# kingdomseed/Deep-Fake-Audio-Classifier

Measured on AMD Instinct MI355X. Metric: utterances/sec fwd (2D-CNN, [B,T=321,F=180]) at 1/2/4/8 GPU; dev EER parity, higher is better.
Workload: dtype bf16; 1 GPU; BASELINE configs[1]: CNN2D eval forward, synthetic [256,321,180] per GPU, bf16 storage / fp32 accumulate, strided view of stored [B,180,321]; batch_per_gpu=256, T=321, F=180, parallelism=utterance-sharded x1, no collective

## Files before the change

deep-fake-audio-classifier_amd/csrc/api.hip:

```cpp
#include <stdlib.h>

#include <algorithm>

#include "dfa_checks.h"

using namespace dfa;

template <typename Fill>
static int stage_ragged_table(dfa_ctx* ctx, const int32_t* lengths, int B, size_t words, void* dst, Fill fill_rest) {
  if (words > ctx->ragged_cap) {
    for (auto& e : ctx->ragged_done)
      if (e) DFA_HIP_CHECK(ctx, hipEventSynchronize(e));
    if (ctx->ragged_host) DFA_HIP_CHECK(ctx, hipHostFree(ctx->ragged_host));
    ctx->ragged_host = nullptr;
    ctx->ragged_cap = 0;
    const size_t cap = std::max(words, (size_t)4 * 256);
    DFA_HIP_CHECK(ctx, hipHostMalloc((void**)&ctx->ragged_host, dfa_ctx::kRaggedSlots * cap * sizeof(int32_t), hipHostMallocDefault));
    ctx->ragged_cap = cap;
  }
  const int slot = ctx->ragged_slot;
  ctx->ragged_slot = (slot + 1) % dfa_ctx::kRaggedSlots;
  if (!ctx->ragged_done[slot]) DFA_HIP_CHECK(ctx, hipEventCreateWithFlags(&ctx->ragged_done[slot], hipEventDisableTiming));
  else DFA_HIP_CHECK(ctx, hipEventSynchronize(ctx->ragged_done[slot]));
  int32_t* tab = ctx->ragged_host + slot * ctx->ragged_cap;
// ... 97 lines not shown

namespace {
__global__ __launch_bounds__(256) void poison_lds_kernel(unsigned pattern, unsigned* sink) {
  extern __shared__ unsigned lds_words[];
  constexpr int N = 160 * 1024 / 4;
  for (int i = threadIdx.x; i < N; i += 256) lds_words[i] = pattern;
  __syncthreads();
  __builtin_amdgcn_s_sleep(127);
  if (lds_words[(threadIdx.x * 97 + blockIdx.x) % N] != pattern) sink[0] = 1;
}
hipError_t launch_poison_lds(dfa_ctx* ctx, unsigned half) {
  hipError_t e = hipSetDevice(ctx->device);
  if (e == hipSuccess) e = hipFuncSetAttribute((const void*)poison_lds_kernel, hipFuncAttributeMaxDynamicSharedMemorySize, 160 * 1024);
  if (e != hipSuccess) return e;
  half &= 0xffffu;
  hipLaunchKernelGGL(poison_lds_kernel, dim3(2048), dim3(256), 160 * 1024, ctx->stream, half | (half << 16), (unsigned*)ctx->zero_page);
  return hipGetLastError();
}
}

namespace {
enum OptionKind { OPT_FLAG, OPT_INT };
struct Option { const char* name; int dfa_ctx::*field; OptionKind kind; };
const Option kOptions[] = {
    {"time_split", &dfa_ctx::time_split, OPT_INT},
    {"conv1_bwd_fused", &dfa_ctx::conv1_bwd_fused, OPT_FLAG}, {"dgrad_m16", &dfa_ctx::dgrad_m16, OPT_FLAG},
    {"conv1_mfma", &dfa_ctx::conv1_mfma, OPT_FLAG}, {"cae_enc1_mfma", &dfa_ctx::cae_enc1_mfma, OPT_FLAG},
    {"cae_enc_dma", &dfa_ctx::cae_enc_dma, OPT_FLAG}, {"cae_dgrad_mfma", &dfa_ctx::cae_dgrad_mfma, OPT_FLAG},
    {"cae_conv_stats", &dfa_ctx::cae_conv_stats, OPT_FLAG}, {"cae_bwd_fold", &dfa_ctx::cae_bwd_fold, OPT_FLAG},
    {"cae_enc4_wide", &dfa_ctx::cae_enc4_wide, OPT_FLAG}, {"cae_dec_fused", &dfa_ctx::cae_dec_fused, OPT_FLAG},
    {"block3_m16", &dfa_ctx::block3_m16, OPT_FLAG}, {"fuse_conv1", &dfa_ctx::fuse_conv1, OPT_FLAG},
    {"fuse_blocks123", &dfa_ctx::fuse_blocks123, OPT_FLAG}, {"persist123", &dfa_ctx::persist123, OPT_FLAG},
    {"lds_pipe", &dfa_ctx::lds_pipe, OPT_FLAG}, {"carry_a1", &dfa_ctx::carry_a1, OPT_FLAG},
    {"phase123", &dfa_ctx::phase123, OPT_FLAG},
};
}

int dfa_ctx_set_option(dfa_ctx* ctx, const char* name, int value) {
  if (!ctx || !name) return DFA_E_NULL_PTR;
  if (strcmp(name, "poison_lds") == 0) {
    hipError_t e = launch_poison_lds(ctx, (unsigned)value);
    return e == hipSuccess ? DFA_OK : fail(ctx, DFA_E_HIP, "poison_lds: %s", hipGetErrorString(e));
  }
  if (strcmp(name, "train_conv_variant") == 0) { set_train_conv_variant(value); return DFA_OK; }
  if (strcmp(name, "wgrad_variant") == 0) { set_wgrad_variant(value); return DFA_OK; }
  if (strcmp(name, "clock_probe") == 0) {
    if (value && !ctx->clock_buf) {
      DFA_HIP_CHECK(ctx, hipSetDevice(ctx->device));
      DFA_HIP_CHECK(ctx, hipMalloc((void**)&ctx->clock_buf, 1024 * 2 * sizeof(long long)));
    }
    if (value) DFA_HIP_CHECK(ctx, hipMemsetAsync(ctx->clock_buf, 0, 1024 * 2 * sizeof(long long), ctx->stream));
    ctx->clock_probe = value ? 1 : 0;
    return DFA_OK;
  }
  if (strcmp(name, "cnn1d_train_x3") == 0) { ctx->cnn1d_train_x3 = (value < 0 || value > 3) ? 1 : value; return DFA_OK; }
  if (strcmp(name, "cnn1d_fused") == 0) { ctx->cnn1d_fused = value < 0 ? 0 : (value > 2 ? 1 : value); return DFA_OK; }
  if (strcmp(name, "conv_dma") == 0) { ctx->conv_dma = value < 0 ? -1 : value; return DFA_OK; }
  for (const Option& o : kOptions)
    if (strcmp(name, o.name) == 0) { ctx->*o.field = (o.kind == OPT_FLAG) ? (value ? 1 : 0) : value; return DFA_OK; }
  return fail(ctx, DFA_E_UNSUPPORTED, "unknown option '%s'", name);
}

int dfa_ctx_timing_enable(dfa_ctx* ctx, int enable) {
  if (!ctx) return DFA_E_NULL_PTR;
  ctx->timing = (enable == 1) ? 0xffffffffu : (unsigned)enable;
  return DFA_OK;
}
// ... 82 lines not shown
```

deep-fake-audio-classifier_amd/csrc/cnn1d_api.hip:

```cpp
#include "dfa_checks.h"
#include "trace.h"

using namespace dfa;

namespace {

struct Cnn1dPlan {
  size_t h1_off, h2_off, pooled_off, total;
};

Cnn1dPlan plan_cnn1d(int B, int T) {
  Cnn1dPlan p;
  size_t off = 0;
  p.h1_off = off;
  off = align_up(off + (size_t)B * 32 * T * sizeof(float), 256);
  p.h2_off = off;
  off = align_up(off + (size_t)B * 64 * T * sizeof(float), 256);
  p.pooled_off = off;
  off = align_up(off + (size_t)B * 128 * sizeof(float), 256);
  p.total = off;
  return p;
}

int cnn1d_forward_front(dfa_ctx* ctx, bool ragged, bool have_ptrs, int x_dtype, int B, int T, int F) {
// ... 57 lines not shown
}

int dfa_cnn1d_forward(dfa_ctx* ctx, const void* x, int x_dtype, int B, int T, int F, int64_t stride_b, int64_t stride_t,
                      int64_t stride_f, float* logits, void* workspace, size_t workspace_bytes) {
  TraceRange trace_("dfa_cnn1d_forward");
  if (!ctx) return DFA_E_NULL_PTR;
  Cnn1dState& m = ctx->cnn1d;
  DFA_TRY(cnn1d_forward_front(ctx, false, x && logits && workspace, x_dtype, B, T, F));
  const Cnn1dPlan pl = plan_cnn1d(B, T);
  DFA_TRY(check_workspace(ctx, workspace, workspace_bytes, pl.total, false));
  char* ws = (char*)workspace;
  float *h1 = (float*)(ws + pl.h1_off), *h2 = (float*)(ws + pl.h2_off), *pooled = (float*)(ws + pl.pooled_off);
  hipStream_t s = ctx->stream;
  const bool off32 = stride_t >= 0 && stride_f >= 0 && (int64_t)(F - 1) * stride_f + (int64_t)(T - 1) * stride_t < ((int64_t)1 << 31);
  if (ctx->cnn1d_fused == 1 && cnn1d_fused_x3_supports(x, stride_b, stride_t, stride_f, T, F)) {
    ScopedSlot ts(ctx, 4);
    DFA_HIP_CHECK(ctx, launch_cnn1d_fused_x3((const float*)x, m.wx[0], m.b[0], m.wx[1], m.b[1], m.wx[2], m.b[2], m.p[18], m.p[19], logits, B, T, F,
                                             s, ctx->clock_probe ? ctx->clock_buf : nullptr));
    return DFA_OK;
  }
  if (ctx->cnn1d_fused && cnn1d_fused_supports(T) && off32) {
    ScopedSlot ts(ctx, 4);
    DFA_HIP_CHECK(ctx, launch_cnn1d_fused((const float*)x, stride_b, stride_t, stride_f, m.wp[0], m.b[0], m.wp[1], m.b[1], m.wp[2], m.b[2],
                                          m.p[18], m.p[19], logits, B, T, F, s, ctx->clock_probe ? ctx->clock_buf : nullptr));
    return DFA_OK;
  }
  { ScopedSlot ts(ctx, 4);
    DFA_HIP_CHECK(ctx, launch_conv1d((const float*)x, stride_b, stride_f, stride_t, m.w[0], m.b[0], h1, B, F, 32, T, false, s)); }
  { ScopedSlot ts(ctx, 5);
    DFA_HIP_CHECK(ctx, launch_conv1d(h1, (int64_t)32 * T, T, 1, m.w[1], m.b[1], h2, B, 32, 64, T, false, s)); }
  { ScopedSlot ts(ctx, 6);
    DFA_HIP_CHECK(ctx, launch_conv1d(h2, (int64_t)64 * T, T, 1, m.w[2], m.b[2], pooled, B, 64, 128, T, true, s)); }
  { ScopedSlot ts(ctx, 7);
    DFA_HIP_CHECK(ctx, launch_linear(pooled, m.p[18], m.p[19], logits, B, 128, s)); }
  return DFA_OK;
}

int dfa_cnn1d_forward_ragged(dfa_ctx* ctx, const void* x, int x_dtype, int B, int T_max, int F, int64_t stride_b, int64_t stride_t,
                             int64_t stride_f, const int32_t* lengths, float* logits, void* workspace, size_t workspace_bytes) {
  TraceRange trace_("dfa_cnn1d_forward_ragged");
  if (!ctx) return DFA_E_NULL_PTR;
  Cnn1dState& m = ctx->cnn1d;
  DFA_TRY(cnn1d_forward_front(ctx, true, x && logits && workspace && lengths, x_dtype, B, T_max, F));
  if (T_max < 3) return fail(ctx, DFA_E_BAD_SHAPE, "T_max=%d is too short: the ragged cnn1d kernel needs T >= 3", T_max);
  DFA_TRY(check_lengths(ctx, lengths, B, 3, T_max));
  if (stride_t != 1)
    return fail(ctx, DFA_E_UNSUPPORTED, "the ragged cnn1d forward takes the channel-major storage only: stride_t=%lld, needs 1", (long long)stride_t);
  if ((F & 3) != 0) return fail(ctx, DFA_E_UNSUPPORTED, "the ragged cnn1d forward needs F %% 4 == 0 (got F=%d)", F);
  DFA_TRY(check_channel_major(ctx, "ragged cnn1d forward", "stride_f", x, stride_b, stride_f, T_max));
  if ((int64_t)F * stride_f >= ((int64_t)1 << 31))
    return fail(ctx, DFA_E_UNSUPPORTED, "the ragged cnn1d forward needs F * stride_f < 2^31 (got %d * %lld)", F, (long long)stride_f);
  if (ctx->cnn1d_fused != 1)
    return fail(ctx, DFA_E_UNSUPPORTED, "the ragged cnn1d forward needs the default option cnn1d_fused=1 (got %d)", ctx->cnn1d_fused);
  if (cnn1d_ragged_segments(3, F, nullptr, nullptr, nullptr, nullptr, 0) < 1)
    return fail(ctx, DFA_E_UNSUPPORTED, "F=%d: the layer-1 weights leave no LDS for a time window", F);
  DFA_TRY(refuse_capture(ctx, "forward"));
  DFA_TRY(check_workspace(ctx, workspace, workspace_bytes, cnn1d_workspace_bytes(B, T_max, true)));
  DFA_TRY(stage_ragged_lengths(ctx, lengths, B, workspace));
  ScopedSlot ts(ctx, 4);
  DFA_HIP_CHECK(ctx, launch_cnn1d_ragged_x3((const float*)x, stride_b, stride_f, (const int*)workspace, m.wx[0], m.b[0], m.wx[1], m.b[1], m.wx[2],
                                            m.b[2], m.p[18], m.p[19], logits, B, T_max, F, ctx->stream,
                                            ctx->clock_probe ? ctx->clock_buf : nullptr));
  return DFA_OK;
}

int dfa_cnn1d_ragged_segments(int T, int F, int* starts, int* lens, int* owned_lo, int* owned_hi, int cap) {
  return cnn1d_ragged_segments(T, F, starts, lens, owned_lo, owned_hi, cap);
// ... 8 lines not shown
```

deep-fake-audio-classifier_amd/csrc/cnn1d_train_api.hip:

```cpp
#include "train_host.h"
#include "trace.h"

using namespace dfa;

namespace {

struct Train1dPlan {
  size_t z[3], h[2], pooled, dpooled, dz[3], dh[2], stats, sums, partial, total;
};

Train1dPlan plan_train1d(int B, int T, int F) {
  Train1dPlan p;
  Bump take;
  const int C[3] = {32, 64, 128};
  for (int l = 0; l < 3; ++l) p.z[l] = take((size_t)B * C[l] * T * 4);
  for (int l = 0; l < 2; ++l) p.h[l] = take((size_t)B * C[l] * T * 4);
  p.pooled = take((size_t)B * 128 * 4);
  p.dpooled = take((size_t)B * 128 * 4);
  for (int l = 0; l < 3; ++l) p.dz[l] = take((size_t)B * C[l] * T * 4);
  for (int l = 0; l < 2; ++l) p.dh[l] = take((size_t)B * C[l] * T * 4);
  p.stats = take((32 + 64 + 128) * 3 * 4);
  p.sums = take((32 + 64 + 128) * 2 * 4);
  const size_t nch = (size_t)cm_chunks(B);
  size_t pb = nch * 128 * 2 * 4;
// ... 84 lines not shown
  m.train_drop = dc; m.train_B = B; m.train_T = T;
  m.train_ragged = lengths ? 1 : 0; m.train_frames = frames;
  char* ws = (char*)workspace;
  float* partial = (float*)(ws + pl.partial);
  const int C[3] = {32, 64, 128}, Cin[3] = {F, 32, 64};
  const int nch = cm_chunks(B);
  for (int l = 0; l < 3; ++l) {
    float* z = (float*)(ws + pl.z[l]);
    const float* const* q = p + 6 * l;
    if (l == 0) {
      if (x3 && conv1d_x3_supports((const float*)x, stride_b, stride_f, stride_t, z, T, F, 32, terms))
        DFA_HIP_CHECK(ctx, launch_conv1d_x3((const float*)x, stride_b, m.wx3[0], q[1], z, B, F, 32, T, terms, s, x3, aug, lens));
      else
        DFA_HIP_CHECK(ctx, launch_conv1d((const float*)x, stride_b, stride_f, stride_t, q[0], q[1], z, B, F, 32, T, false, s, false, aug, lens));
    } else {
      const float* hin = (const float*)(ws + pl.h[l - 1]);
      if (x3 && conv1d_x3_supports(hin, (int64_t)Cin[l] * T, T, 1, z, T, Cin[l], C[l], terms))
        DFA_HIP_CHECK(ctx, launch_conv1d_x3(hin, (int64_t)Cin[l] * T, m.wx3[l], q[1], z, B, Cin[l], C[l], T, terms, s, x3));
      else
        DFA_HIP_CHECK(ctx, launch_conv1d(hin, (int64_t)Cin[l] * T, T, 1, q[0], q[1], z, B, Cin[l], C[l], T, false, s, false));
    }
    BnStats st = st1d(ws, pl, l);
    const bool shifted = !ctx->bn_sync.fn;
    DFA_HIP_CHECK(ctx, launch_cm_stats(z, partial, B, C[l], T, s, lens, shifted));
    DFA_TRY(finalize_bn_stats(ctx, partial, nch, C[l], frames, st, update_running_stats ? (float*)q[4] : nullptr,
                              update_running_stats ? (float*)q[5] : nullptr, momentum, nullptr, shifted ? z : nullptr, T));
    if (l < 2) {
      dc.layer = 1 + l;
      DFA_HIP_CHECK(ctx, launch_cm_bn_relu_drop(z, st.mean, st.invstd, q[2], q[3], (float*)(ws + pl.h[l]), B, C[l], T, dc, s, lens));
    } else {
      DFA_HIP_CHECK(ctx, launch_cm_bn_relu_meant(z, st.mean, st.invstd, q[2], q[3], (float*)(ws + pl.pooled), B, 128, T, s, lens));
    }
  }
  DFA_HIP_CHECK(ctx, launch_linear((const float*)(ws + pl.pooled), p[18], p[19], logits, B, 128, s));
  return DFA_OK;
}

int cnn1d_backward_impl(dfa_ctx* ctx, int ragged, const void* x, int x_dtype, int B, int T, int F, int64_t stride_b, int64_t stride_t,
                        int64_t stride_f, const float* dlogits, float* const* grads, int ngrads, void* workspace,
                        size_t workspace_bytes) {
  Cnn1dState& m = ctx->cnn1d;
  Train1dPlan pl;
  DFA_TRY(check_backward(ctx, {ragged ? "dfa_cnn1d_backward_ragged" : "dfa_cnn1d_backward",
                               ragged ? "dfa_cnn1d_forward_train_ragged" : "dfa_cnn1d_forward_train", "cnn1d", 14, "dlogits", true},
                         m.train_packed && m.train_B == B && m.train_T == T && m.train_ragged == ragged, x, x_dtype, dlogits, grads, ngrads,
                         workspace, workspace_bytes, [&] { return (pl = plan_train1d(B, T, F)).total + (ragged ? ragged1d_tab_bytes(B) : 0); }));
  if (ragged && ctx->bn_sync.fn)
    return fail(ctx, DFA_E_UNSUPPORTED, "the ragged cnn1d training step cannot run under synchronised BatchNorm (dfa_ctx_set_bn_sync is armed)");
  char* ws = (char*)workspace;
  const int* lens = ragged ? (const int*)(ws + pl.total) : nullptr;
  float* partial = (float*)(ws + pl.partial);
  const float* const* p = m.p;
  hipStream_t s = ctx->stream;
  DropCfg dc = m.train_drop;
  const int C[3] = {32, 64, 128}, Cin[3] = {F, 32, 64};
  float* dpooled = (float*)(ws + pl.dpooled);
  DFA_HIP_CHECK(ctx, launch_linear_bwd(dlogits, p[18], (const float*)(ws + pl.pooled), dpooled, grads[12], grads[13], B, 128, s));
  for (int l = 2; l >= 0; --l) {
    const float* const* q = p + 6 * l;
    BnStats st = st1d(ws, pl, l);
    float* sm = sums1d(ws, pl, l);
    float* dz = (float*)(ws + pl.dz[l]);
    const float* up = (l == 2) ? dpooled : (const float*)(ws + pl.dh[l]);
    dc.layer = 1 + l;
    DFA_HIP_CHECK(ctx, launch_cm_bn_bwd(l == 2 ? 0 : 1, (const float*)(ws + pl.z[l]), st.mean, st.invstd, q[2], q[3], up, partial, sm, dz,
                                        B, C[l], T, dc, s, ctx->bn_sync.fn ? &ctx->bn_sync : nullptr, lens, m.train_frames));
    DFA_HIP_CHECK(ctx, launch_split_sums(sm, grads[4 * l + 2], grads[4 * l + 3], C[l], s));
// ... 75 lines not shown
```

deep-fake-audio-classifier_amd/csrc/cnn2d_api.hip:

```cpp
#include <algorithm>

#include "dfa_checks.h"
#include "trace.h"

using namespace dfa;

namespace {

constexpr int kMaxSeg = 4;

constexpr int kSlots = 512;
constexpr int kSlotsSplit2 = 768;
constexpr int kSlotsSplit3 = 256;
constexpr int kStripCols = c123::SW;
constexpr int kStripColsMfma = 32;

int seg_iters_for(int niter, int nwg, int slots, int period, int forced) {
  if (forced == 0 || niter <= period) return 0;
  int seg;
  if (forced > 0) seg = (niter + forced - 1) / forced;
  else {
    if (nwg >= slots) return 0;
    seg = (int)(((long long)niter * nwg + slots - 1) / slots);
  }
// ... 199 lines not shown
    a.in = a1; a.wpack = m.c2.wpack; a.bias = m.c2.bias; a.out = a2; a.emb = nullptr;
    a.B = B; a.H = pl.H1; a.W = F; a.COUT = 64; a.inv_h = 0.f; a.relu = 1; a.zero_page = ctx->zero_page;
    a.seg_iters = pl.seg12;
    if (prec == DFA_PREC_BF16X3) DFA_HIP_CHECK(ctx, launch_cnn2d_block2_split(a, s, ctx->lds_pipe));
    else DFA_HIP_CHECK(ctx, launch_cnn2d_block2(prec, a, s, ctx->conv_dma, ctx->lds_pipe));
  }
  if (pl.path != DFA_CNN2D_PATH_CONV123) {
    ScopedSlot ts(ctx, 2);
    ConvArgs a{};
    a.in = a2; a.wpack = m.c3.wpack; a.bias = m.c3.bias; a.out = nullptr; a.emb = emb;
    a.B = B; a.H = pl.H2; a.W = F; a.COUT = 128; a.inv_h = 1.0f / (float)pl.H2; a.relu = 1; a.zero_page = ctx->zero_page;
    a.chunk_iters = pl.chunk3;
    a.seg_iters = pl.seg3;
    if (pl.seg3) {
      a.emb_seg_stride = (size_t)B * 128 * F;
      a.emb = (float*)(ws + pl.emb_off) + a.emb_seg_stride;
    }
    if (prec == DFA_PREC_BF16X3) {
      DFA_HIP_CHECK(ctx, launch_cnn2d_block3_split(a, s, ctx->lds_pipe));
    } else if (prec == DFA_PREC_BF16 && ctx->block3_m16) {
      a.wpack = m.c3_m16;
      a.clock_stamps = ctx->clock_probe ? ctx->clock_buf : nullptr;
      DFA_HIP_CHECK(ctx, launch_cnn2d_block3_m16(a, s, ctx->lds_pipe));
    } else {
      DFA_HIP_CHECK(ctx, launch_cnn2d_block3(prec, a, s, ctx->conv_dma, ctx->lds_pipe));
    }
  }
  {
    ScopedSlot ts(ctx, 3);
    if (pl.nseg3 > 1) {
      const size_t n = (size_t)B * 128 * F;
      DFA_HIP_CHECK(ctx, launch_emb_reduce((const float*)(ws + pl.emb_off) + n, pl.nseg3, n, n, 1.0f / (float)pl.H2, emb, s));
    }
    DFA_HIP_CHECK(ctx, launch_linear(emb, m.p[18], m.p[19], logits, B, 128 * F, s));
  }
  return DFA_OK;
}

int dfa_cnn2d_forward_ragged(dfa_ctx* ctx, const void* x, int x_dtype, int B, int T_max, int F, int64_t stride_b, int64_t stride_t,
                             int64_t stride_f, const int32_t* lengths, float* logits, float* embedding, void* workspace,
                             size_t workspace_bytes) {
  TraceRange trace_("dfa_cnn2d_forward_ragged");
  if (!ctx) return DFA_E_NULL_PTR;
  Cnn2dState& m = ctx->cnn2d;
  DFA_TRY(cnn2d_forward_front(ctx, true, x && logits && workspace && lengths, x_dtype, B, T_max, F));
  DFA_TRY(check_lengths(ctx, lengths, B, 4, T_max));
  const int prec = m.prepared_prec;
  if (prec != DFA_PREC_BF16)
    return fail(ctx, DFA_E_UNSUPPORTED, "the ragged forward has kernels for precision bf16 only (prepared: %d)", prec);
  if (!ctx->fuse_conv1 || !ctx->block3_m16)
    return fail(ctx, DFA_E_UNSUPPORTED, "the ragged forward needs the default options fuse_conv1=1 and block3_m16=1");
  DFA_TRY(refuse_capture(ctx, "forward"));
  const Cnn2dForwardPlan pl = plan_for(ctx, B, T_max, F, prec, true);
  DFA_TRY(cnn2d_forward_buffers(ctx, workspace, workspace_bytes, pl.total, embedding));
  char* ws = (char*)workspace;
  const int* dtab = (const int*)(ws + pl.tab_off);
  hipStream_t s = ctx->stream;
  int nseg3 = 1;
  std::vector<int32_t> extra((size_t)2 * B);
  for (int b = 0; b < B; ++b) {
    const int h2 = lengths[b] / 4, niter3 = (h2 + 1) / 2, chunk = chunk3_for(niter3);
    const float inv_h = 1.0f / (float)h2;
    memcpy(&extra[b], &inv_h, 4);
    extra[B + b] = chunk;
    nseg3 = std::max(nseg3, (niter3 + chunk - 1) / chunk);
  }
  DFA_TRY(stage_ragged_lengths_extra(ctx, lengths, B, extra.data(), extra.size(), ws + pl.tab_off));
  const RaggedTab rt{dtab, B};
  void* a2 = ws + pl.a2_off;
  float* emb = embedding ? embedding : (float*)(ws + pl.emb_off);
  {
    ScopedSlot ts(ctx, 1);
    DFA_HIP_CHECK(ctx, launch_conv12_ragged(x, x_dtype, stride_b, stride_t, stride_f, m.c1pack, m.c1bias, m.c2.wpack, m.c2.bias, a2,
                                            B, T_max, F, dtab, s, ctx->lds_pipe, pl.seg12));
  }
  {
    ScopedSlot ts(ctx, 2);
    ConvArgs a{};
    a.in = a2; a.wpack = m.c3_m16; a.bias = m.c3.bias; a.out = nullptr; a.emb = emb;
    a.B = B; a.H = pl.H2; a.W = F; a.COUT = 128; a.relu = 1; a.zero_page = ctx->zero_page;
    a.chunk_iters = 1;
    if (pl.split3) {
      a.seg_iters = pl.seg3;
      a.emb_seg_stride = (size_t)B * 128 * F;
      a.emb = (float*)(ws + pl.emb_off) + a.emb_seg_stride;
    }
    DFA_HIP_CHECK(ctx, launch_cnn2d_block3_m16_ragged(a, rt, nseg3, s, ctx->lds_pipe));
  }
  {
    ScopedSlot ts(ctx, 3);
    if (pl.split3) {
      const size_t n = (size_t)B * 128 * F;
      DFA_HIP_CHECK(ctx, launch_emb_reduce_ragged((const float*)(ws + pl.emb_off) + n, n, 128 * F, dtab, B, emb, s));
    }
    DFA_HIP_CHECK(ctx, launch_linear(emb, m.p[18], m.p[19], logits, B, 128 * F, s));
  }
  return DFA_OK;
}

}
```

deep-fake-audio-classifier_amd/csrc/conv123_body.h:

```cpp
#ifndef DFA_CONV123_BODY_SCOPE
#error "conv123_body.h holds kernel bodies: include it only from conv123_fused.hip, conv123_persist.hip, conv123_carry.hip and conv123_phase.hip"
#endif
#ifndef DFA_CONV123_BODY_H
#define DFA_CONV123_BODY_H
#include "dfa_internal.h"
#ifdef DFA_STAMPS
#include <algorithm>
#include <climits>
#include <cstdio>
#include <vector>
#endif

#ifndef DFA_C123_PRIO
#define DFA_C123_PRIO 0
#endif
#ifndef DFA_C123_CBAR
#define DFA_C123_CBAR 4
#endif
#ifndef DFA_C123_CARRY
#define DFA_C123_CARRY 0
#endif

namespace dfa {

// ... 365 lines not shown
    c1_issue(st, j);
    if constexpr (PIPE) asm volatile("s_waitcnt lgkmcnt(0)" : "+v"(st.w0), "+v"(st.w1), "+v"(st.w2), "+v"(st.w3));
    c1_mfma(st, std::integral_constant<int, 0>{});
    c1_relu(st, j, std::integral_constant<int, 0>{});
    c1_store(st, ringblk, std::integral_constant<int, 0>{});
    c1_mfma(st, std::integral_constant<int, 1>{});
    c1_relu(st, j, std::integral_constant<int, 1>{});
    c1_store(st, ringblk, std::integral_constant<int, 1>{});
  };
  auto produce_fresh = [&](int j, int ringblk) {
#if DFA_C123_CARRY
    produce_cy(j, ringblk, std::true_type{});
    return;
#endif
    C1State st;
    c1_issue(st, j);
    if constexpr (PIPE) asm volatile("s_waitcnt lgkmcnt(0)" : "+v"(st.w0), "+v"(st.w1), "+v"(st.w2), "+v"(st.w3));
    c1_mfma(st, std::integral_constant<int, 0>{});
    c1_relu(st, j, std::integral_constant<int, 0>{});
    c1_store_fresh(st, ringblk, std::integral_constant<int, 0>{});
    c1_mfma(st, std::integral_constant<int, 1>{});
    c1_relu(st, j, std::integral_constant<int, 1>{});
    c1_store_fresh(st, ringblk, std::integral_constant<int, 1>{});
  };

  const int col = f0 - 1 + r;
  bool col_ok = col >= 0 && col < W;
  const int a2_dst = r * CPB;
  const int a2_sw = r & 6;
  auto lds_drain = [&]() { if constexpr (PIPE) asm volatile("s_waitcnt lgkmcnt(0)" ::: "memory"); };
  auto barrier = [&]() { lds_drain(); __syncthreads(); };

  barrier();
  x_load(0); x_store(0);
  x_load(1); x_store(1);
  barrier();
  produce_now(0, 0);
  produce_now(1, 1);
  barrier();
  x_load(2); x_store(0);
  barrier();

  auto unit = [&](auto ph_c, auto rp_c, int it) {
    constexpr int PH = decltype(ph_c)::value, RPI = decltype(rp_c)::value;
    f32x16_t acc0, acc1;
    constexpr int NR = 12 * NKG;
    constexpr int S_RELU0 = 9 * NKG + 2;
    constexpr int S_BAR = 4;
    constexpr int C_MFMA = 5, C_XLOAD = 7, C_RELU = 10, C_MFMA1 = 11, C_STORE = 13, C_RELU1 = 17, C_XSTORE = 19, C_STORE1 = 21;
    constexpr int NWR = CARRY ? 2 : 4;
    constexpr int N_STORE = CARRY ? 6 : 2, C_CARRY = C_STORE + PF;
    static_assert(C_CARRY == C_RELU1 && C_CARRY + PF - 1 < C_STORE1 + PF - 1 && C_CARRY < NR, "");
    u32x4_t xbuf[PF];
    C1State c1;
#if DFA_C123_CARRY
    u32x4_t cy0, cy2;
#endif
    auto step = [&](auto s_c) {
      constexpr int s = decltype(s_c)::value;
      if constexpr (s < NR) {
        constexpr int i = s / (3 * NKG), dx = (s / NKG) % 3, kg = s % NKG;
        constexpr int ringrow = (BR * PH + 2 * RPI + i) % (3 * BR);
        xbuf[s % PF] = lds_frag<ringrow * ROWB, PIPE>(plds + (xa[dx] ^ (kg << 5)));
        if constexpr (s == S_BAR) {
          if constexpr (PIPE) asm volatile("s_barrier" ::: "memory");
          else __syncthreads();
          c1_issue(c1, it + 2);
        }
      }
      if constexpr (s >= PF - 1) {
        constexpr int c = s - (PF - 1);
        constexpr int i = c / (3 * NKG), dx = (c / NKG) % 3, kg = c % NKG;
        constexpr int young_r = (NR - 1 - c) < (PF - 1) ? (NR - 1 - c) : (PF - 1);
        constexpr int C_ST2 = CARRY ? C_CARRY : C_STORE1;
// ... 416 lines not shown
```

deep-fake-audio-classifier_amd/csrc/dfa_internal.h:

```cpp
#pragma once
#include <hip/hip_runtime.h>
#include <stdint.h>
#include <stdarg.h>
#include <stdio.h>
#include <string.h>

#include <algorithm>
#include <vector>

#include "../../include/dfa_hip.h"
#include "conv3x3_mfma.h"
#include "conv123_host.h"
#include "rng.h"

namespace dfa {

constexpr float kBnEps = 1e-5f;

constexpr int kMaxSlots = 16;
constexpr int kEventsPerSlot = 256;

struct SlotTimer {
  std::vector<hipEvent_t> start, stop;
  int used = 0;
// ... 82 lines not shown
struct DlqState {
  const float* p[DFA_DLQ_NPARAMS] = {nullptr};
  bool have_params = false;
  bool prepared = false;
  int in_ch = 0;
  void* packed = nullptr;
  void* w[3] = {nullptr, nullptr, nullptr};
  float* b[3] = {nullptr, nullptr, nullptr};
  void* train_packed = nullptr;
  void* tw[5] = {nullptr, nullptr, nullptr, nullptr, nullptr};
  int tw_in_ch = 0;
  int train_B = 0, train_T = 0;
  DropCfg train_drop{};
};

}

struct dfa_ctx {
  int device = 0;
  hipStream_t stream = nullptr;
  char err[512] = {0};
  void* zero_page = nullptr;
  dfa::BnSync bn_sync;
  int block3_m16 = 1;
  int fuse_conv1 = 1;
  int fuse_blocks123 = 1;
  int persist123 = 1;
  int carry_a1 = 1;
  int phase123 = 1;
  int last_conv123_phase = 0;
  int last_conv123_form = 0;
  int num_cus = 0;
  int lds_pipe = 1;
  int time_split = -1;
  int conv1_bwd_fused = 1;
  int conv1_mfma = 1;
  int dgrad_m16 = 1;
  int cae_enc1_mfma = 1;
  int cae_enc_dma = 1;
  int cae_dgrad_mfma = 1;
  int cae_conv_stats = 1;
  int cae_bwd_fold = 1;
  int cae_enc4_wide = 1;
  int cae_dec_fused = 1;
  int cnn1d_train_x3 = 1;
  int cnn1d_fused = 1;
  int clock_probe = 0;
  long long* clock_buf = nullptr;
  float* aug_keep = nullptr;
  int aug_keep_cap = 0, aug_keep_slot = 0;
  float* mse_partial = nullptr;
  double* clip_partial = nullptr;
  static constexpr int kRaggedSlots = 4;
  int32_t* ragged_host = nullptr;
  size_t ragged_cap = 0;
  int ragged_slot = 0;
  hipEvent_t ragged_done[kRaggedSlots] = {};
  int conv_dma = -1;
  dfa::Cnn2dState cnn2d;
  dfa::Cnn1dState cnn1d;
  dfa::CaeState cae;
  dfa::DlqState dlq;
  unsigned timing = 0;
  dfa::SlotTimer slots[dfa::kMaxSlots];
};

// ... 28 lines not shown
    if ((int)t.start.size() <= t.used) {
      hipEvent_t a, b;
      if (hipEventCreate(&a) != hipSuccess || hipEventCreate(&b) != hipSuccess) return;
      t.start.push_back(a);
      t.stop.push_back(b);
    }
    idx = t.used++;
    (void)hipEventRecord(t.start[idx], ctx->stream);
  }
  ~ScopedSlot() {
    if (idx >= 0) (void)hipEventRecord(ctx->slots[slot].stop[idx], ctx->stream);
  }
};

hipError_t launch_fold_conv1(const float* w, const float* b, const float* g, const float* beta, const float* mean,
                             const float* var, float* w1, float* b1, int cout, hipStream_t s);
hipError_t launch_fold_pack_conv3x3(const float* w, const float* b, const float* g, const float* beta,
                                    const float* mean, const float* var, int cin_total, int cin_off, int cin, int cout,
                                    int prec, uint4* wpack, float* bias, hipStream_t s, int fold = 1,
                                    float post_scale = 1.0f);
hipError_t launch_pack_conv3x3_dgrad(const float* w, int cin, int cout, int co_off, int co_n, int prec, uint4* wpack,
                                     float* bias, hipStream_t s);
hipError_t launch_fold_pack_convt2x2(const float* w, const float* b, const float* g, const float* beta,
                                     const float* mean, const float* var, int cin, int cout, int prec, uint4* wpack,
                                     float* bias, hipStream_t s, int fold = 1);
hipError_t launch_gemm_tn_bf16(const void* X, const void* Z, float* partial, size_t partial_floats, int M, int N, int K,
                               int* nparts, hipStream_t s);
hipError_t launch_gemm_f32(int a_bf16, const void* A, int64_t sam, int64_t sak, int b_bf16, const void* Bm, int64_t sbk,
                           int64_t sbn, float* C, int M, int N, int K, int ksplit, hipStream_t s);
hipError_t launch_conv1(const void* x, int x_dtype, int64_t sb, int64_t st, int64_t sf, const float* w1,
                        const float* b1, void* out, int out_prec, int B, int T, int F, hipStream_t s,
                        const DropCfg* drop = nullptr, const AugCfg* aug = nullptr);
hipError_t launch_linear(const float* emb, const float* w, const float* bias, float* logits, int B, int K,
                         hipStream_t s);
hipError_t launch_emb_reduce(const float* parts, int nparts, size_t stride, size_t n, float inv_h, float* out, hipStream_t s);
hipError_t launch_emb_reduce_ragged(const float* parts, size_t stride, int per_b, const int* tab, int B, float* out, hipStream_t s);
hipError_t launch_fold_conv1d(const float* w, const float* b, const float* g, const float* beta, const float* mean,
                              const float* var, float* wf, float* bf, int cin, int cout, hipStream_t s);
hipError_t launch_cae_enc1_mfma(const void* x, int x_dtype, int64_t sb, int64_t st, int64_t sf, const float* mu, const float* sigma,
                                const uint4* c1pack, const float* c1bias, void* out, int B, int T, int F, hipStream_t s);
hipError_t launch_cae_enc1_mfma_ragged(const void* x, int x_dtype, int64_t sb, int64_t st, int64_t sf, const float* mu, const float* sigma,
                                       const uint4* c1pack, const float* c1bias, void* out, int B, int T, int F, const int* tab,
                                       hipStream_t s);
hipError_t launch_pack_cae_enc1_mfma(const float* w1, const float* b1, uint4* pack, float* bias, hipStream_t s);
int cae_dec_fused_tiles(int H4, int W4);
hipError_t launch_cae_opad_consts(const float* b2, const uint4* wp3, const float* b3, const float* w4, const float* b4, float* cst,
                                  hipStream_t s);
hipError_t launch_cae_dec_fused(const void* lat, const uint4* wp1, const float* b1, const uint4* wp2, const float* b2, const uint4* wp3,
                                const float* b3, const float* w4, const float* b4, const uint4* w4pack, const float* cst, const void* x,
                                int x_dtype, int64_t sb, int64_t st, int64_t sf, const float* mu, const float* sigma, float* recon,
                                float* partial, int B, int H4, int W4, int T, int F, hipStream_t s, long long* stamps = nullptr);
hipError_t launch_cae_dec_fused_ragged(const void* lat, const uint4* wp1, const float* b1, const uint4* wp2, const float* b2,
                                       const uint4* wp3, const float* b3, const float* w4, const float* b4, const uint4* w4pack,
                                       const float* cst, const void* x, int x_dtype, int64_t sb, int64_t st, int64_t sf, const float* mu,
                                       const float* sigma, float* partial, int B, int H4, int W4, int T, int F, const int* tab,
                                       hipStream_t s);
bool cae_dec_fused_supports(int T, int F, int64_t st, int64_t sf);
hipError_t launch_pack_cae_dec4(const float* w4, uint4* pack, hipStream_t s);
hipError_t launch_cae_mse_finalize(const float* partial, int nblk, float inv_n, float* mse, int B, hipStream_t s);
hipError_t launch_cae_mse_finalize_ragged(const float* partial, int nblk, const int* tab, float* mse, int B, hipStream_t s);
int cnn1d_fused_ncp_pad(int cin, int layer);
size_t cnn1d_fused_pack_floats(int cin, int cout, int layer);
bool cnn1d_fused_supports(int T);
hipError_t launch_pack_cnn1d_fused(const float* wf, float* wp, int cin, int cout, int layer, hipStream_t s);
hipError_t launch_cnn1d_fused(const float* x, int64_t sb, int64_t st, int64_t sf, const float* wp1, const float* b1, const float* wp2,
                              const float* b2, const float* wp3, const float* b3, const float* cw, const float* cb, float* logits, int B,
                              int T, int F, hipStream_t s, long long* stamps = nullptr);
// ... 229 lines not shown
```

deep-fake-audio-classifier_amd/csrc/linear.hip:

```cpp
#include "dfa_internal.h"

namespace dfa {

__global__ __launch_bounds__(256) void linear1_kernel(const float* __restrict__ emb, const float* __restrict__ w,
                                                      const float* __restrict__ bias, float* __restrict__ logits,
                                                      int K) {
  __shared__ float part[4];
  const int b = blockIdx.x, tid = threadIdx.x;
  const float* e = emb + (size_t)b * K;
  float acc = 0.f;
  const int K4 = ((((uintptr_t)e | (uintptr_t)w) & 15) == 0) ? (K >> 2) : 0;
  for (int j = tid; j < K4; j += 256) {
    const float4 ev = reinterpret_cast<const float4*>(e)[j], wv = reinterpret_cast<const float4*>(w)[j];
    acc = fmaf(ev.x, wv.x, acc);
    acc = fmaf(ev.y, wv.y, acc);
    acc = fmaf(ev.z, wv.z, acc);
    acc = fmaf(ev.w, wv.w, acc);
  }
  for (int j = 4 * K4 + tid; j < K; j += 256) acc = fmaf(e[j], w[j], acc);
#pragma unroll
  for (int off = 32; off > 0; off >>= 1) acc += __shfl_down(acc, off, 64);
  if ((tid & 63) == 0) part[tid >> 6] = acc;
  __syncthreads();
  if (tid == 0) logits[b] = ((part[0] + part[1]) + (part[2] + part[3])) + bias[0];
}

hipError_t launch_linear(const float* emb, const float* w, const float* bias, float* logits, int B, int K,
                         hipStream_t s) {
  hipLaunchKernelGGL(linear1_kernel, dim3(B), dim3(256), 0, s, emb, w, bias, logits, K);
  return hipGetLastError();
}

__global__ __launch_bounds__(256) void emb_reduce_kernel(const float* __restrict__ parts, int nparts, size_t stride, size_t n,
                                                         float inv_h, float* __restrict__ out) {
  const size_t i = ((size_t)blockIdx.x * 256 + threadIdx.x) * 4;
  if (i + 3 < n) {
    float4 v = make_float4(0.f, 0.f, 0.f, 0.f);
    for (int k = 0; k < nparts; ++k) {
      const float4 p = *reinterpret_cast<const float4*>(parts + (size_t)k * stride + i);
      v.x += p.x; v.y += p.y; v.z += p.z; v.w += p.w;
    }
    *reinterpret_cast<float4*>(out + i) = make_float4(v.x * inv_h, v.y * inv_h, v.z * inv_h, v.w * inv_h);
  } else {
    for (size_t j = i; j < n; ++j) {
      float v = 0.f;
      for (int k = 0; k < nparts; ++k) v += parts[(size_t)k * stride + j];
      out[j] = v * inv_h;
    }
  }
}

hipError_t launch_emb_reduce(const float* parts, int nparts, size_t stride, size_t n, float inv_h, float* out, hipStream_t s) {
  const size_t nthreads = (n + 3) / 4;
  hipLaunchKernelGGL(emb_reduce_kernel, dim3((unsigned)((nthreads + 255) / 256)), dim3(256), 0, s, parts, nparts, stride, n, inv_h, out);
  return hipGetLastError();
}

__global__ __launch_bounds__(256) void emb_reduce_ragged_kernel(const float* __restrict__ parts, size_t stride, int per_b,
                                                                const int* __restrict__ tab, int B, float* __restrict__ out) {
  const size_t i = ((size_t)blockIdx.x * 256 + threadIdx.x) * 4;
  if (i >= (size_t)B * per_b) return;
  const int b = (int)(i / per_b);
// ... 19 lines not shown
```

deep-fake-audio-classifier_amd/csrc/train_api.hip:

```cpp
#include "train_host.h"
#include "trace.h"

using namespace dfa;

namespace {

struct TrainPlan {
  int H1, H2;
  size_t a1, z2, a2, z3, emb, demb, msum, dz3, da2, dz2, da1, raw, stats, sums, partial, partial_bytes, total;
};

TrainPlan plan_train(int B, int T, int F, int prec) {
  TrainPlan p;
  const size_t es = (prec == DFA_PREC_BF16) ? 2 : 4;
  p.H1 = T / 2;
  p.H2 = p.H1 / 2;
  Bump take;
  p.a1 = take((size_t)B * p.H1 * F * 32 * es);
  p.z2 = take((size_t)B * p.H1 * F * 64 * es);
  p.a2 = take((size_t)B * p.H2 * F * 64 * es);
  p.z3 = take((size_t)B * p.H2 * F * 128 * es);
  p.emb = take((size_t)B * 128 * F * 4);
  p.demb = take((size_t)B * 128 * F * 4);
  p.msum = take((size_t)B * 128 * F * 2 * 4);
// ... 104 lines not shown
  DFA_TRY(conv1_train_stats(ctx, conv1_block(m, x, x_dtype, stride_b, stride_t, stride_f, B, T, F, ws, pl, dc), m.train_c1_mfma, m.train_c1_fused,
                            rm[0], rv[0], momentum));
  dc.layer = 1;
  if (m.train_c1_mfma)
    DFA_HIP_CHECK(ctx, launch_conv1_mfma(C1X_FWD, x, stride_b, stride_t, stride_f, m.tw1, m.tb1, ws + pl.a1, nullptr, nullptr, B, T, F, dc, s));
  else
  DFA_HIP_CHECK(ctx, launch_conv1(x, x_dtype, stride_b, stride_t, stride_f, m.tw1, m.tb1, ws + pl.a1, prec, B, T, F, s, &dc, aug));
  const int nstrips = (F + 31) / 32;
  {
    ConvArgs a = conv_args(ws + pl.a1, m.t2, ws + pl.z2, B, pl.H1, F, 64, ctx);
    a.stats_partial = partial;
    DFA_HIP_CHECK(ctx, launch_train_fwd2(prec, a, s));
  }
  BnStats s2 = stat_ptrs(ws, pl, 1);
  DFA_TRY(finalize_bn_stats(ctx, partial, B * nstrips, 64, (double)B * pl.H1 * F, s2, rm[1], rv[1], momentum, partial + (size_t)B * nstrips * 128));
  dc.layer = 2;
  DFA_HIP_CHECK(ctx, launch_bn_relu_pool_drop(prec, ws + pl.z2, s2.mean, s2.invstd, p[8], p[9], ws + pl.a2, B, pl.H1, F, 64, dc, s));
  {
    ConvArgs a = conv_args(ws + pl.a2, m.t3, ws + pl.z3, B, pl.H2, F, 128, ctx);
    a.stats_partial = partial;
    if (fwd3_m16) {
      a.wpack = t3_m16;
      DFA_HIP_CHECK(ctx, launch_train_fwd3_m16(a, s, train_conv_variant() == 2));
    } else {
      DFA_HIP_CHECK(ctx, launch_train_fwd3(prec, a, s));
    }
  }
  BnStats s3 = stat_ptrs(ws, pl, 2);
  const int np3 = B * (fwd3_m16 ? (F + 29) / 30 : nstrips);
  DFA_TRY(finalize_bn_stats(ctx, partial, np3, 128, (double)B * pl.H2 * F, s3, rm[2], rv[2], momentum, partial + (size_t)np3 * 256));
  float* emb = (float*)(ws + pl.emb);
  DFA_HIP_CHECK(ctx, launch_bn_relu_meant(prec, ws + pl.z3, s3.mean, s3.invstd, p[14], p[15], emb, B, pl.H2, F, 128, s, (float*)(ws + pl.msum)));
  if (embedding) DFA_HIP_CHECK(ctx, hipMemcpyAsync(embedding, emb, (size_t)B * 128 * F * 4, hipMemcpyDeviceToDevice, s));
  DFA_HIP_CHECK(ctx, launch_linear(emb, p[18], p[19], logits, B, 128 * F, s));
  return DFA_OK;
}

int dfa_cnn2d_backward(dfa_ctx* ctx, const void* x, int x_dtype, int B, int T, int F, int64_t stride_b, int64_t stride_t,
                       int64_t stride_f, const float* dlogits, float* const* grads, int ngrads, void* workspace,
                       size_t workspace_bytes) {
  TraceRange trace_("dfa_cnn2d_backward");
  if (!ctx) return DFA_E_NULL_PTR;
  Cnn2dState& m = ctx->cnn2d;
  const int prec = m.train_prec;
  TrainPlan pl;
  DFA_TRY(check_backward(ctx, {"dfa_cnn2d_backward", "dfa_cnn2d_forward_train", "cnn2d", 14, "dlogits", false},
                         m.train_packed && m.train_B == B && m.train_T == T, x, x_dtype, dlogits, grads, ngrads, workspace, workspace_bytes,
                         [&] { return (pl = plan_train(B, T, F, prec)).total; }));
  char* ws = (char*)workspace;
  float* partial = (float*)(ws + pl.partial);
  const float* const* p = m.p;
  hipStream_t s = ctx->stream;
  DropCfg dc = m.train_drop;
  BnStats s2 = stat_ptrs(ws, pl, 1), s3 = stat_ptrs(ws, pl, 2);
  float *sm2 = sums_ptr(ws, pl, 1), *sm3 = sums_ptr(ws, pl, 2);
  float* demb = (float*)(ws + pl.demb);
  const dfa::BnSync* sync = ctx->bn_sync.fn ? &ctx->bn_sync : nullptr;
  DFA_HIP_CHECK(ctx, launch_linear_bwd(dlogits, p[18], (const float*)(ws + pl.emb), demb, grads[12], grads[13], B, 128 * F, s, 128, F));
  DFA_HIP_CHECK(ctx, launch_bn_bwd_meant_saved(prec, ws + pl.z3, s3.mean, s3.invstd, p[14], p[15], demb, (const float*)(ws + pl.msum), partial,
                                               sm3, ws + pl.dz3, B, pl.H2, F, 128, s, sync));
  DFA_HIP_CHECK(ctx, launch_split_sums(sm3, grads[10], grads[11], 128, s));
  DFA_HIP_CHECK(ctx, launch_wgrad3x3(prec, 64, 128, ws + pl.dz3, ws + pl.a2, partial, grads[8], grads[9], B, pl.H2, F, kWgradWGs, s));
  DFA_HIP_CHECK(ctx, launch_dgrad3(m.train_dgrad_m16, prec, conv_args(ws + pl.dz3, m.d3, ws + pl.da2, B, pl.H2, F, 64, ctx), (float*)(ws + pl.raw), s));
  dc.layer = 2;
  {
    int ppb_;
    float* scratch2 = partial + (size_t)bn_bwd_blocks(B, pl.H1, F, &ppb_) * 64 * 2;
// ... 96 lines not shown
```

Baseline: 442,300 utterances/s.

## Batch float4 loads in final linear kernel and carry x prologue loads in registers

Rewrites the per-utterance linear head kernel to issue many float4 loads of embedding and weight before accumulating, raising memory-level parallelism for the K=128*F dot product. The old serial kernel stays available behind a new linear_inflight option, which defaults to on. Separately, under a DFA_C123_CARRY compile flag, the conv123 prologue loads three input rows into registers up front instead of alternating load and store. The batched loads cost more registers, and the summation order changes slightly.

```diff
diff --git a/deep-fake-audio-classifier_amd/csrc/api.hip b/deep-fake-audio-classifier_amd/csrc/api.hip
--- a/deep-fake-audio-classifier_amd/csrc/api.hip
+++ b/deep-fake-audio-classifier_amd/csrc/api.hip
@@ -153,7 +153,7 @@
     {"block3_m16", &dfa_ctx::block3_m16, OPT_FLAG}, {"fuse_conv1", &dfa_ctx::fuse_conv1, OPT_FLAG},
     {"fuse_blocks123", &dfa_ctx::fuse_blocks123, OPT_FLAG}, {"persist123", &dfa_ctx::persist123, OPT_FLAG},
     {"lds_pipe", &dfa_ctx::lds_pipe, OPT_FLAG}, {"carry_a1", &dfa_ctx::carry_a1, OPT_FLAG},
-    {"phase123", &dfa_ctx::phase123, OPT_FLAG},
+    {"phase123", &dfa_ctx::phase123, OPT_FLAG}, {"linear_inflight", &dfa_ctx::linear_inflight, OPT_FLAG},
 };
 }
 
diff --git a/deep-fake-audio-classifier_amd/csrc/cnn1d_api.hip b/deep-fake-audio-classifier_amd/csrc/cnn1d_api.hip
--- a/deep-fake-audio-classifier_amd/csrc/cnn1d_api.hip
+++ b/deep-fake-audio-classifier_amd/csrc/cnn1d_api.hip
@@ -113,7 +113,7 @@
   { ScopedSlot ts(ctx, 6);
     DFA_HIP_CHECK(ctx, launch_conv1d(h2, (int64_t)64 * T, T, 1, m.w[2], m.b[2], pooled, B, 64, 128, T, true, s)); }
   { ScopedSlot ts(ctx, 7);
-    DFA_HIP_CHECK(ctx, launch_linear(pooled, m.p[18], m.p[19], logits, B, 128, s)); }
+    DFA_HIP_CHECK(ctx, launch_linear(pooled, m.p[18], m.p[19], logits, B, 128, s, ctx->linear_inflight)); }
   return DFA_OK;
 }
 
diff --git a/deep-fake-audio-classifier_amd/csrc/cnn1d_train_api.hip b/deep-fake-audio-classifier_amd/csrc/cnn1d_train_api.hip
--- a/deep-fake-audio-classifier_amd/csrc/cnn1d_train_api.hip
+++ b/deep-fake-audio-classifier_amd/csrc/cnn1d_train_api.hip
@@ -140,7 +140,7 @@
       DFA_HIP_CHECK(ctx, launch_cm_bn_relu_meant(z, st.mean, st.invstd, q[2], q[3], (float*)(ws + pl.pooled), B, 128, T, s, lens));
     }
   }
-  DFA_HIP_CHECK(ctx, launch_linear((const float*)(ws + pl.pooled), p[18], p[19], logits, B, 128, s));
+  DFA_HIP_CHECK(ctx, launch_linear((const float*)(ws + pl.pooled), p[18], p[19], logits, B, 128, s, ctx->linear_inflight));
   return DFA_OK;
 }
 
diff --git a/deep-fake-audio-classifier_amd/csrc/cnn2d_api.hip b/deep-fake-audio-classifier_amd/csrc/cnn2d_api.hip
--- a/deep-fake-audio-classifier_amd/csrc/cnn2d_api.hip
+++ b/deep-fake-audio-classifier_amd/csrc/cnn2d_api.hip
@@ -255,7 +255,7 @@
       const size_t n = (size_t)B * 128 * F;
       DFA_HIP_CHECK(ctx, launch_emb_reduce((const float*)(ws + pl.emb_off) + n, pl.nseg3, n, n, 1.0f / (float)pl.H2, emb, s));
     }
-    DFA_HIP_CHECK(ctx, launch_linear(emb, m.p[18], m.p[19], logits, B, 128 * F, s));
+    DFA_HIP_CHECK(ctx, launch_linear(emb, m.p[18], m.p[19], logits, B, 128 * F, s, ctx->linear_inflight));
   }
   return DFA_OK;
 }
@@ -316,9 +316,9 @@
       const size_t n = (size_t)B * 128 * F;
       DFA_HIP_CHECK(ctx, launch_emb_reduce_ragged((const float*)(ws + pl.emb_off) + n, n, 128 * F, dtab, B, emb, s));
     }
-    DFA_HIP_CHECK(ctx, launch_linear(emb, m.p[18], m.p[19], logits, B, 128 * F, s));
-  }
-  return DFA_OK;
-}
-
-}
+    DFA_HIP_CHECK(ctx, launch_linear(emb, m.p[18], m.p[19], logits, B, 128 * F, s, ctx->linear_inflight));
+  }
+  return DFA_OK;
+}
+
+}
diff --git a/deep-fake-audio-classifier_amd/csrc/conv123_body.h b/deep-fake-audio-classifier_amd/csrc/conv123_body.h
--- a/deep-fake-audio-classifier_amd/csrc/conv123_body.h
+++ b/deep-fake-audio-classifier_amd/csrc/conv123_body.h
@@ -421,6 +421,36 @@
   auto barrier = [&]() { lds_drain(); __syncthreads(); };
 
   barrier();
+#if DFA_C123_CARRY
+  {
+    unsigned short xr0[NXLD], xr1[NXLD];
+    bool xk0[NXLD], xk1[NXLD];
+    x_load(0);
+#pragma unroll
+    for (int k = 0; k < NXLD; ++k) { xr0[k] = xreg[k]; xk0[k] = xok[k]; }
+    x_load(1);
+#pragma unroll
+    for (int k = 0; k < NXLD; ++k) { xr1[k] = xreg[k]; xk1[k] = xok[k]; }
+    x_load(2);
+#pragma unroll
+    for (int k = 0; k < NXLD; ++k) {
+      const unsigned short v2 = xreg[k]; const bool k2 = xok[k];
+      xreg[k] = xr0[k]; xok[k] = xk0[k]; xr0[k] = v2; xk0[k] = k2;
+    }
+    x_store(0);
+#pragma unroll
+    for (int k = 0; k < NXLD; ++k) { xreg[k] = xr1[k]; xok[k] = xk1[k]; }
+    x_store(1);
+    barrier();
+    produce_now(0, 0);
+    produce_now(1, 1);
+    barrier();
+#pragma unroll
+    for (int k = 0; k < NXLD; ++k) { xreg[k] = xr0[k]; xok[k] = xk0[k]; }
+    x_store(0);
+    barrier();
+  }
+#else
   x_load(0); x_store(0);
   x_load(1); x_store(1);
   barrier();
@@ -429,6 +459,7 @@
   barrier();
   x_load(2); x_store(0);
   barrier();
+#endif
 
   auto unit = [&](auto ph_c, auto rp_c, int it) {
     constexpr int PH = decltype(ph_c)::value, RPI = decltype(rp_c)::value;
diff --git a/deep-fake-audio-classifier_amd/csrc/dfa_internal.h b/deep-fake-audio-classifier_amd/csrc/dfa_internal.h
--- a/deep-fake-audio-classifier_amd/csrc/dfa_internal.h
+++ b/deep-fake-audio-classifier_amd/csrc/dfa_internal.h
@@ -138,6 +138,7 @@
   int last_conv123_form = 0;
   int num_cus = 0;
   int lds_pipe = 1;
+  int linear_inflight = 1;
   int time_split = -1;
   int conv1_bwd_fused = 1;
   int conv1_mfma = 1;
@@ -232,7 +233,7 @@
                         const float* b1, void* out, int out_prec, int B, int T, int F, hipStream_t s,
                         const DropCfg* drop = nullptr, const AugCfg* aug = nullptr);
 hipError_t launch_linear(const float* emb, const float* w, const float* bias, float* logits, int B, int K,
-                         hipStream_t s);
+                         hipStream_t s, int inflight);
 hipError_t launch_emb_reduce(const float* parts, int nparts, size_t stride, size_t n, float inv_h, float* out, hipStream_t s);
 hipError_t launch_emb_reduce_ragged(const float* parts, size_t stride, int per_b, const int* tab, int B, float* out, hipStream_t s);
 hipError_t launch_fold_conv1d(const float* w, const float* b, const float* g, const float* beta, const float* mean,
diff --git a/deep-fake-audio-classifier_amd/csrc/linear.hip b/deep-fake-audio-classifier_amd/csrc/linear.hip
--- a/deep-fake-audio-classifier_amd/csrc/linear.hip
+++ b/deep-fake-audio-classifier_amd/csrc/linear.hip
@@ -2,9 +2,53 @@
 
 namespace dfa {
 
+__device__ __forceinline__ void linear1_finish(float acc, const float* __restrict__ bias, float* __restrict__ logits, int b,
+                                               int tid) {
+  __shared__ float part[4];
+#pragma unroll
+  for (int off = 32; off > 0; off >>= 1) acc += __shfl_down(acc, off, 64);
+  if ((tid & 63) == 0) part[tid >> 6] = acc;
+  __syncthreads();
+  if (tid == 0) logits[b] = ((part[0] + part[1]) + (part[2] + part[3])) + bias[0];
+}
+
+constexpr int kLinearBatch = 24;
+
 __global__ __launch_bounds__(256) void linear1_kernel(const float* __restrict__ emb, const float* __restrict__ w,
                                                       const float* __restrict__ bias, float* __restrict__ logits,
                                                       int K) {
+  constexpr int NB = kLinearBatch;
+  const int b = blockIdx.x, tid = threadIdx.x;
+  const float* e = emb + (size_t)b * K;
+  float acc = 0.f;
+  const int K4 = ((((uintptr_t)e | (uintptr_t)w) & 15) == 0) ? (K >> 2) : 0;
+  const float4* e4 = reinterpret_cast<const float4*>(e);
+  const float4* w4 = reinterpret_cast<const float4*>(w);
+  for (int j = tid; j < K4; j += NB * 256) {
+    float4 ev[NB], wv[NB];
+#pragma unroll
+    for (int i = 0; i < NB; ++i) {
+      const int jj = j + i * 256;
+      if (jj < K4) { ev[i] = e4[jj]; wv[i] = w4[jj]; }
+      else { ev[i] = make_float4(0.f, 0.f, 0.f, 0.f); wv[i] = ev[i]; }
+    }
+#pragma unroll
+    for (int i = 0; i < NB; ++i) {
+      if (j + i * 256 < K4) {
+        acc = fmaf(ev[i].x, wv[i].x, acc);
+        acc = fmaf(ev[i].y, wv[i].y, acc);
+        acc = fmaf(ev[i].z, wv[i].z, acc);
+        acc = fmaf(ev[i].w, wv[i].w, acc);
+      }
+    }
+  }
+  for (int t = 4 * K4 + tid; t < K; t += 256) acc = fmaf(e[t], w[t], acc);
+  linear1_finish(acc, bias, logits, b, tid);
+}
+
+__global__ __launch_bounds__(256) void linear1_serial_kernel(const float* __restrict__ emb, const float* __restrict__ w,
+                                                             const float* __restrict__ bias, float* __restrict__ logits,
+                                                             int K) {
   __shared__ float part[4];
   const int b = blockIdx.x, tid = threadIdx.x;
   const float* e = emb + (size_t)b * K;
@@ -26,8 +70,9 @@
 }
 
 hipError_t launch_linear(const float* emb, const float* w, const float* bias, float* logits, int B, int K,
-                         hipStream_t s) {
-  hipLaunchKernelGGL(linear1_kernel, dim3(B), dim3(256), 0, s, emb, w, bias, logits, K);
+                         hipStream_t s, int inflight) {
+  if (inflight) hipLaunchKernelGGL(linear1_kernel, dim3(B), dim3(256), 0, s, emb, w, bias, logits, K);
+  else hipLaunchKernelGGL(linear1_serial_kernel, dim3(B), dim3(256), 0, s, emb, w, bias, logits, K);
   return hipGetLastError();
 }
 
diff --git a/deep-fake-audio-classifier_amd/csrc/train_api.hip b/deep-fake-audio-classifier_amd/csrc/train_api.hip
--- a/deep-fake-audio-classifier_amd/csrc/train_api.hip
+++ b/deep-fake-audio-classifier_amd/csrc/train_api.hip
@@ -160,7 +160,7 @@
   float* emb = (float*)(ws + pl.emb);
   DFA_HIP_CHECK(ctx, launch_bn_relu_meant(prec, ws + pl.z3, s3.mean, s3.invstd, p[14], p[15], emb, B, pl.H2, F, 128, s, (float*)(ws + pl.msum)));
   if (embedding) DFA_HIP_CHECK(ctx, hipMemcpyAsync(embedding, emb, (size_t)B * 128 * F * 4, hipMemcpyDeviceToDevice, s));
-  DFA_HIP_CHECK(ctx, launch_linear(emb, p[18], p[19], logits, B, 128 * F, s));
+  DFA_HIP_CHECK(ctx, launch_linear(emb, p[18], p[19], logits, B, 128 * F, s, ctx->linear_inflight));
   return DFA_OK;
 }
 
```

Measured after the change: 443,200 utterances/s, median of 6. About the same (+0.2%).
